# yweweler/single-speaker-tts

Hardware: AMD Instinct MI355X
Metric: mel-frames/sec (end-to-end text->waveform incl. 60-iter Griffin-Lim, 64-utt LJ-Speech-shaped batch per GPU) (higher is better)
Workload: dtype f32

## Files before the change

single-speaker-tts_amd/csrc/api_handle.hip:

```cpp
#include "api_internal.h"

namespace tts_api {
thread_local std::string g_create_error;
const char* const kStageNames[ST_COUNT] = {"encoder", "decoder", "postnet", "denorm", "gl_iter", "gl_final", "debug_gemm", "eval_loss", "features"};
}

namespace tts_api {


int fail(tts_handle_t h, int code, const std::string& msg) {
    if (h) h->err = msg;
    else g_create_error = msg;
    return code;
}


const char* kAtt = "decoder2/decoder/output_projection_wrapper/multi_rnn_cell/cell_0/attention_wrapper";

const char* kMrc = "decoder2/decoder/output_projection_wrapper/multi_rnn_cell";


std::string bn_name(int i) {
    return i == 0 ? std::string("batch_normalization") : "batch_normalization_" + std::to_string(i);
}
// ... 571 lines not shown
        if (h->hio.ids_dev[i]) hipFree(h->hio.ids_dev[i]);
        if (h->hio.wav_pinned[i]) hipHostFree(h->hio.wav_pinned[i]);
        if (h->hio.wav_dev[i]) hipFree(h->hio.wav_dev[i]);
        if (i == 0) {
            for (auto& kv : h->glg.tw) hipFree(kv.second);
            if (h->glg.window) hipFree(h->glg.window);
            if (h->glg.rwss) hipFree(h->glg.rwss);
        }
        if (h->hio.lin_pinned[i]) hipHostFree(h->hio.lin_pinned[i]);
        if (h->hio.lin_dev[i]) hipFree(h->hio.lin_dev[i]);
        if (h->hio.ali_pinned[i]) hipHostFree(h->hio.ali_pinned[i]);
        if (h->hio.ali_dev[i]) hipFree(h->hio.ali_dev[i]);
        if (h->hio.ev_h2d[i]) hipEventDestroy(h->hio.ev_h2d[i]);
        if (h->hio.ev_enc[i]) hipEventDestroy(h->hio.ev_enc[i]);
        if (h->hio.ev_ready[i]) hipEventDestroy(h->hio.ev_ready[i]);
        if (h->hio.ev_d2h[i]) hipEventDestroy(h->hio.ev_d2h[i]);
    }
    if (h->hio.status_pinned) hipHostFree(h->hio.status_pinned);
    if (h->hio.out) hipStreamDestroy(h->hio.out);
    if (h->ev_aux) hipEventDestroy(h->ev_aux);
    if (h->ev_front_done) hipEventDestroy(h->ev_front_done);
    for (int i = 0; i < 2; ++i) {
        if (h->ev_enc_ready[i]) hipEventDestroy(h->ev_enc_ready[i]);
        if (h->ev_dec_done[i]) hipEventDestroy(h->ev_dec_done[i]);
        if (h->ev_gap[i]) hipEventDestroy(h->ev_gap[i]);
    }
    if (h->encs) hipStreamDestroy(h->encs);
    if (h->ev_serial_done) hipEventDestroy(h->ev_serial_done);
    if (h->ev_graph_done) hipEventDestroy(h->ev_graph_done);
    for (int i = 0; i < 2; ++i) {
        if (h->ev_post_done[i]) hipEventDestroy(h->ev_post_done[i]);
        if (h->ev_gl_done[i]) hipEventDestroy(h->ev_gl_done[i]);
    }
    if (h->own_stream) hipStreamDestroy(h->stream);
    delete h;
    return TTS_OK;
}


const char* tts_last_error(tts_handle_t h) { return h ? h->err.c_str() : g_create_error.c_str(); }


int tts_set_stream(tts_handle_t h, void* s) {
    DeviceScope dev_scope(h);
    if (!h) return TTS_ERR_INVALID;
    {
        int rc = sync_all(h);
        if (rc) return rc;
    }
    h->post_pending[0] = h->post_pending[1] = false;
    h->gl_pending[0] = h->gl_pending[1] = false;
    h->gl_wide_used[0] = h->gl_wide_used[1] = false;
    {
        int rc = graph_drop(h);
        if (rc) return rc;
    }
    if (h->own_stream) hipStreamDestroy(h->stream);
    if (s) {
        h->stream = reinterpret_cast<hipStream_t>(s);
        h->own_stream = false;
    } else {
        HIPCHK(h, hipStreamCreate(&h->stream));
        h->own_stream = true;
    }
    return TTS_OK;
}


int tts_set_option(tts_handle_t h, const char* key, int value) {
    DeviceScope dev_scope(h);
    if (!h || !key) return TTS_ERR_INVALID;
    if (!std::strcmp(key, "use_graph")) {
        int have = 0;
        if (value && !(value == 2 && h->debug_hooks) && !graph_runtime_ok(&have))
            return fail(h, TTS_ERR_UNSUPPORTED,
                        "use_graph: this process runs the library on HIP runtime " + std::to_string(have) + ", older than the " +
                        std::to_string(HIP_VERSION) + " it was built with (a libamdhip64 loaded before the library, e.g. the one "
                        "PyTorch bundles); hipGraph replays of the decoder are wrong there (csrc/api_internal.h, `use_graph`) -- the "
                        "launches are enqueued directly instead");
        h->use_graph = value;
    }
    else if (!std::strcmp(key, "profile")) h->profile = value;
    else if (!std::strcmp(key, "fused_tail")) h->fused_tail = value;
    else if (!std::strcmp(key, "persistent_decoder")) {
        if (value != h->persistent_decoder) {
            int rc = sync_all(h);
            if (rc) return rc;
        }
        h->persistent_decoder = value;
    }
    else if (!std::strcmp(key, "gl_pair")) h->gl_pair = value;
    else if (!std::strcmp(key, "gl_wide_from")) h->gl_wide = value < -2 ? -2 : value;
    else if (!std::strcmp(key, "pd_ws")) {
        if (value != h->pd_ws) {
            int rc = sync_all(h);
            if (rc) return rc;
        }
        h->pd_ws = value;
    }
    else if (!std::strcmp(key, "enc_stream")) {
        int rc = sync_all(h);
        if (rc) return rc;
        h->enc_stream = value;
    }
    else if (!std::strcmp(key, "debug_hooks")) h->debug_hooks = value;
    else if (!std::strcmp(key, "pd_debug_delay") || !std::strcmp(key, "gl_runs") || !std::strcmp(key, "gl_run_len") ||
             !std::strcmp(key, "timeline") || !std::strcmp(key, "gl_workers") || !std::strcmp(key, "pd_rows")) {
        if (!h->debug_hooks && value != 0)
            return fail(h, TTS_ERR_INVALID, std::string(key) + ": a test hook; set the option \"debug_hooks\" to 1 on this handle first");
        if (!std::strcmp(key, "pd_debug_delay")) h->pd_debug_delay = value;
        else if (!std::strcmp(key, "gl_runs")) h->gl_runs = value;
        else if (!std::strcmp(key, "gl_run_len")) h->gl_run_len = value;
        else if (!std::strcmp(key, "gl_workers")) h->gl_workers = value;
        else if (!std::strcmp(key, "pd_rows")) h->pd_rows = value;
        else h->timeline = value;
    }
    else if (!std::strcmp(key, "reserve_cus")) {
        if (value != h->reserve_cus) {
            int rc = sync_all(h);
            if (rc) return rc;
        }
        h->reserve_cus = value;
    } else if (!std::strcmp(key, "hold_lds_kb")) {
        if (value < 1 || value > 160) return fail(h, TTS_ERR_INVALID, "hold_lds_kb must be 1..160");
        h->hold_lds_kb = value;
    } else if (!std::strcmp(key, "pipeline")) {
        int rc = sync_all(h);
        if (rc) return rc;
        h->post_pending[0] = h->post_pending[1] = false;
        h->gl_pending[0] = h->gl_pending[1] = false;
        h->gl_wide_used[0] = h->gl_wide_used[1] = false;
        h->pipeline = value;
    }
    else return fail(h, TTS_ERR_INVALID, std::string("unknown option ") + key);
    return TTS_OK;
}


int tts_synchronize(tts_handle_t h) {
    DeviceScope dev_scope(h);
    if (!h) return TTS_ERR_INVALID;
    return sync_all(h);
}


int tts_manifest_size(tts_handle_t h) { return h ? (int)h->manifest.size() : TTS_ERR_INVALID; }


int tts_manifest_entry(tts_handle_t h, int i, const char** name, int64_t shape[4], int* ndim) {
    if (!h || i < 0 || i >= (int)h->manifest.size()) return TTS_ERR_INVALID;
    const auto& e = h->manifest[i];
    if (name) *name = e.name.c_str();
    if (ndim) *ndim = (int)e.shape.size();
    if (shape)
        for (size_t d = 0; d < 4; ++d) shape[d] = d < e.shape.size() ? e.shape[d] : 1;
    return TTS_OK;
}


int tts_set_weight(tts_handle_t h, const char* name, const float* data, const int64_t* shape, int ndim) {
    if (!h || !name || !data || !shape) return TTS_ERR_INVALID;
    for (const auto& e : h->manifest) {
        if (e.name != name) continue;
        if ((int)e.shape.size() != ndim) return fail(h, TTS_ERR_INVALID, std::string("rank mismatch for ") + name);
        for (int d = 0; d < ndim; ++d)
            if (e.shape[d] != shape[d]) return fail(h, TTS_ERR_INVALID, std::string("shape mismatch for ") + name);
// ... 280 lines not shown
```

single-speaker-tts_amd/csrc/api_internal.h:

```cpp
#pragma once
#include <cmath>
#include <cstdio>
#include <cstring>
#include <memory>
#include <mutex>
#include <string>
#include <utility>
#include <vector>
#include "decoder.h"
#include "griffin_lim.h"
#include "tts_common.h"
#include <algorithm>
#include <map>

namespace tts_api {
using namespace tts;


extern thread_local std::string g_create_error;

struct ManifestEntry {
    std::string name;
    std::vector<int64_t> shape;
    size_t numel() const {
        size_t n = 1;
        for (auto d : shape) n *= (size_t)d;
        return n;
    }
};

struct CbhgWeights {
    int n_banks = 0, n_filters = 0, c_in = 0, proj_filters[2] = {0, 0};
    std::vector<const float*> bank_wt, bank_b, bank_scale, bank_shift;
    const float* proj_wt[2];
    const float* proj_b[2];
    const float* proj_scale[2];
    const float* proj_shift[2];
    const float* lifter_wt;
    const float* lifter_b;
    std::vector<const float*> hw_wt, hw_b;
    const float* gru_in_wt;
    const float* gru_in_b;
    const float* gru_rec;
};

enum Stage { ST_ENCODER = 0, ST_DECODER, ST_POSTNET, ST_DENORM, ST_GL_ITER, ST_GL_FINAL, ST_DEBUG_GEMM, ST_EVAL_LOSS, ST_FEATURES, ST_COUNT };
extern const char* const kStageNames[ST_COUNT];

struct ProfSpan {
    hipEvent_t a, b;
    int stage;
    int64_t launches;
};


}
using namespace tts_api;

struct tts_handle_s {
    tts_config_t cfg;
    int device = 0;
    hipStream_t stream = nullptr;
    bool own_stream = false;
    std::string err;
    int use_graph = 0;
    int fused_tail = 1;
    bool tail_configured = false;
    int profile = 0;
    int pipeline = 1;
    int reserve_cus = 32;
    int hold_lds_kb = 64;
    hipStream_t aux = nullptr;
    int* hold_flags = nullptr;
    hipEvent_t ev_aux = nullptr;
    unsigned call_count = 0;
    hipStream_t front = nullptr;
    hipStream_t encs = nullptr;
    int enc_stream = 1;
    hipEvent_t ev_enc_ready[2] = {nullptr, nullptr};
    hipEvent_t ev_dec_done[2] = {nullptr, nullptr};
    hipEvent_t ev_gap[2] = {nullptr, nullptr};
    bool enc_ready_pending[2] = {false, false}, dec_done_pending[2] = {false, false}, gap_pending[2] = {false, false};
    hipEvent_t ev_front_done = nullptr;
    hipEvent_t ev_post_done[2] = {nullptr, nullptr};
    bool post_pending[2] = {false, false};
    bool gl_wide_used[2] = {false, false};
    hipEvent_t ev_gl_done[2] = {nullptr, nullptr};
    bool gl_pending[2] = {false, false};
    bool front_pending = false;
    hipEvent_t ev_serial_done = nullptr;
    bool serial_pending = false;
    unsigned syn_calls = 0;
    int syn_shape[3] = {0, 0, 0};
    int last_enc_ahead = -1;
    bool in_synthesize = false;
    int persistent_decoder = 1;
    int pd_ws = 1;
    bool ws_configured = false;
    int gl_pair = 3;
    int gl_wide = -1;
    int n_cus_dev = 0;
    bool pd_configured = false;
    int debug_hooks = 0;
    int pd_debug_delay = 0;
    int gl_runs = 0;
    int gl_run_len = 0;
    int timeline = 0;
    int gl_workers = 0;
    unsigned* gl_ring = nullptr;
    unsigned gl_ring_seq = 0;
    unsigned* gl_ring_last = nullptr;
    hipStream_t gl_ring_stream = nullptr;
    float* pre_keys = nullptr;
    bool pd_used = false;
    unsigned* pd_sync = nullptr;
    int pd_clusters = 0;
    int* cur_hold_flag = nullptr;
    int cur_cu_budget = 0;
    bool dec_chip_idle = false;
    int pd_rows = 0;
    int pd_rows_used = 0;

    struct {
        hipStream_t out = nullptr;
        int32_t* ids_pinned[3] = {nullptr, nullptr, nullptr};
        int32_t* ids_dev[3] = {nullptr, nullptr, nullptr};
        size_t ids_bytes = 0;
        float* wav_dev[3] = {nullptr, nullptr, nullptr};
        float* wav_pinned[3] = {nullptr, nullptr, nullptr};
        size_t wav_bytes = 0;
        hipEvent_t ev_h2d[3] = {nullptr, nullptr, nullptr};
        hipEvent_t ev_enc[3] = {nullptr, nullptr, nullptr};
        hipEvent_t ev_ready[3] = {nullptr, nullptr, nullptr};
        hipEvent_t ev_d2h[3] = {nullptr, nullptr, nullptr};
        bool d2h_pending[3] = {false, false, false}, enc_pending[3] = {false, false, false};
        size_t n_floats[3] = {0, 0, 0};
        float* lin_dev[3] = {nullptr, nullptr, nullptr};
        float* lin_pinned[3] = {nullptr, nullptr, nullptr};
        size_t lin_bytes = 0;
        float* ali_dev[3] = {nullptr, nullptr, nullptr};
        float* ali_pinned[3] = {nullptr, nullptr, nullptr};
        size_t ali_bytes = 0;
        size_t n_lin[3] = {0, 0, 0}, n_ali[3] = {0, 0, 0};
        bool failed[3] = {false, false, false};
        int* status_pinned = nullptr;
        int tickets = 0;
    } hio;
    bool defer_projection = false, has_pending_proj = false;
    int defer_parity = 0;
// ... 189 lines not shown
```

single-speaker-tts_amd/csrc/api_stages.hip:

```cpp
#include "api_internal.h"

namespace tts_api {


int run_cbhg(tts_handle_t h, const CbhgWeights& w, const char* tag, const float* x, int B, int T, float* out,
             int64_t* launches) {
    const tts_config_t& c = h->cfg;
    const int M = B * T;
    const int NB = w.n_banks, NF = w.n_filters;
    const int U = c.n_highway_units, H = c.n_gru_units;
    const std::string t(tag);
    WS(h, (t + ".bank").c_str(), float, (size_t)M * NB * NF, bank);
    WS(h, (t + ".p1").c_str(), float, (size_t)M * w.proj_filters[0], p1);
    WS(h, (t + ".p2").c_str(), float, (size_t)M * w.proj_filters[1], p2);
    WS(h, (t + ".hw0").c_str(), float, (size_t)M * U, hw0);
    WS(h, (t + ".hw1").c_str(), float, (size_t)M * U, hw1);
    WS(h, (t + ".xproj").c_str(), float, (size_t)M * 6 * H, xproj);

    for (int k0 = 0; k0 < NB; k0 += TTS_GEMM_MAX_GROUPS) {
        GemmBatch b;
        std::memset(&b, 0, sizeof(b));
        const int ng = std::min(TTS_GEMM_MAX_GROUPS, NB - k0);
        for (int i = 0; i < ng; ++i) {
            const int k = k0 + ng - 1 - i;
            b.g[i] = conv_group(x, w.c_in, k + 1, T, w.bank_wt[k], w.bank_b[k], w.bank_scale[k], w.bank_shift[k], bank,
                                NB * NF, k * NF, M, NF, ACT_RELU, 0);
        }
        HIPCHK(h, launch_gemm(h->stream, b, ng));
        ++*launches;
    }
    {
        GemmGroup g = conv_group(bank, NB * NF, 3, T, w.proj_wt[0], w.proj_b[0], w.proj_scale[0], w.proj_shift[0], p1,
                                 w.proj_filters[0], 0, M, w.proj_filters[0], ACT_RELU, 1);
        const int slices = gemm_splitk_slices(g.K);
        if (slices > 1) {
            WS(h, (t + ".splitk").c_str(), float, (size_t)slices * M * g.N, part);
            HIPCHK(h, launch_gemm_splitk(h->stream, g, slices, part));
            ++*launches;
        } else {
            int rc = run_single(h, g);
            if (rc) return rc;
        }
        ++*launches;
    }
    {
        GemmGroup g = conv_group(p1, w.proj_filters[0], 3, T, w.proj_wt[1], w.proj_b[1], w.proj_scale[1],
                                 w.proj_shift[1], p2, w.proj_filters[1], 0, M, w.proj_filters[1], ACT_NONE, 0);
        g.R = x;
        g.ldr = w.c_in;
        int rc = run_single(h, g);
        if (rc) return rc;
        ++*launches;
    }
    if (h->fused_tail && cbhg_tail_supports(w.proj_filters[1], U, H, (int)w.hw_wt.size(), M)) {
        if (!h->tail_configured) {
            HIPCHK(h, cbhg_tail_configure());
            h->tail_configured = true;
        }
        CbhgTailParams tp;
        std::memset(&tp, 0, sizeof(tp));
        tp.X = p2; tp.ldx = w.proj_filters[1]; tp.c_in = w.proj_filters[1];
        tp.lifter_wt = w.lifter_wt; tp.lifter_b = w.lifter_b;
        tp.n_hw = (int)w.hw_wt.size();
        for (int l = 0; l < tp.n_hw; ++l) { tp.hw_wt[l] = w.hw_wt[l]; tp.hw_b[l] = w.hw_b[l]; }
        tp.gru_wt = w.gru_in_wt; tp.gru_b = w.gru_in_b;
        tp.hw_out = hw0; tp.xproj = xproj; tp.M = M;
        HIPCHK(h, launch_cbhg_tail(h->stream, tp));
        ++*launches;
    } else {
        {
            int rc = run_single(h, dense_group(p2, w.proj_filters[1], w.lifter_wt, w.lifter_b, hw0, U, M, U,
                                               w.proj_filters[1], ACT_RELU));
            if (rc) return rc;
            ++*launches;
        }
        float* cur = hw0;
        float* nxt = hw1;
        for (size_t l = 0; l < w.hw_wt.size(); ++l) {
            GemmGroup g = dense_group(cur, U, w.hw_wt[l], w.hw_b[l], nxt, U, M, 2 * U, U, ACT_NONE);
            g.epi = EPI_HIGHWAY;
            int rc = run_single(h, g);
            if (rc) return rc;
            ++*launches;
            std::swap(cur, nxt);
        }
        {
            int rc = run_single(h, dense_group(cur, U, w.gru_in_wt, w.gru_in_b, xproj, 6 * H, M, 6 * H, U, ACT_NONE));
            if (rc) return rc;
            ++*launches;
        }
    }
    HIPCHK(h, launch_bigru(h->stream, xproj, 6 * H, w.gru_rec, out, B, T, H, c.force_cudnn));
    ++*launches;
    return TTS_OK;
}


int check_ready(tts_handle_t h) {
    if (!h) return TTS_ERR_INVALID;
    if (!h->finalized) return fail(h, TTS_ERR_NOT_LOADED, "weights not loaded: call tts_finalize_weights first");
    return TTS_OK;
}


int gl_tables(tts_handle_t h) {
    auto& g = h->gl;
    if (g.configured) return TTS_OK;
    HIPCHK(h, gl_configure());
    std::vector<float2> t1(1024), t2(1024);
    for (int k = 0; k < 1024; ++k) {
        const double a1 = -2.0 * M_PI * k / 1024.0, a2 = -2.0 * M_PI * k / 2048.0;
        t1[k] = make_float2((float)std::cos(a1), (float)std::sin(a1));
        t2[k] = make_float2((float)std::cos(a2), (float)std::sin(a2));
    }
    HIPCHK(h, hipMalloc(&g.tw1024, 1024 * sizeof(float2)));
    HIPCHK(h, hipMalloc(&g.tw2048, 1024 * sizeof(float2)));
    HIPCHK(h, hipMemcpy(g.tw1024, t1.data(), 1024 * sizeof(float2), hipMemcpyHostToDevice));
    HIPCHK(h, hipMemcpy(g.tw2048, t2.data(), 1024 * sizeof(float2), hipMemcpyHostToDevice));
    {
        std::vector<float2> tb(1024 + 15 * 64);
        for (int k = 0; k < 1024; ++k) tb[k] = t2[k];
        for (int i = 0; i < 15 * 64; ++i) tb[1024 + i] = t1[(i & 63) * ((i >> 6) + 1)];
        HIPCHK(h, hipMalloc(&g.tables, tb.size() * sizeof(float2)));
        HIPCHK(h, hipMemcpy(g.tables, tb.data(), tb.size() * sizeof(float2), hipMemcpyHostToDevice));
    }
    {
        hipDeviceProp_t prop;
        HIPCHK(h, hipGetDeviceProperties(&prop, h->device));
        g.n_cus = prop.multiProcessorCount > 0 ? prop.multiProcessorCount : 256;
    }
    g.configured = true;
    return TTS_OK;
}


int device_cus(tts_handle_t h) { return h->gl.n_cus; }


int gl_fp(int n_fft);

int glg_prepare(tts_handle_t h, int T, int win, int hop, int n_fft);

int glg_twiddles(tts_handle_t h, int n_fft, const float2** out);


int stft_prepare(tts_handle_t h, int n, int win, int hop, int n_fft) {
    if (n_fft != TTS_GL_NFFT) return fail(h, TTS_ERR_UNSUPPORTED, "stft: n_fft != 2048 takes the general kernels (stft_run)");
    if (win < 2 || win > n_fft || hop < 1) return fail(h, TTS_ERR_INVALID, "stft: need 2 <= win_length <= n_fft, hop >= 1");
    if (n <= n_fft / 2) return fail(h, TTS_ERR_INVALID, "stft: signal shorter than n_fft/2 (reflect padding undefined)");
// ... 951 lines not shown
```

single-speaker-tts_amd/csrc/cbhg_tail.hip:

```cpp
#include "tts_common.h"

namespace tts {

#define CT_BM 128
#define CT_U 128
#define CT_XLD (CT_U + 4)
#define CT_BK 32
#define CT_BLD (CT_BK + 4)
#define CT_BN 256
#define CT_THREADS 512

#define CT_AIMG (3 * CT_BM * 64)
#define CT_BIMG (3 * CT_BN * 64)
size_t cbhg_tail_lds_bytes() { return (size_t)CT_BM * CT_XLD * sizeof(float) + CT_AIMG + CT_BIMG; }
typedef __bf16 ct_bf16x8_t __attribute__((ext_vector_type(8)));
__device__ __forceinline__ void ct_split3(float x, unsigned& h, unsigned& m, unsigned& l) {
    h = __float_as_uint(x);
    const float r1 = x - __uint_as_float(h & 0xFFFF0000u);
    m = __float_as_uint(r1);
    const float r2 = r1 - __uint_as_float(m & 0xFFFF0000u);
    l = __float_as_uint(r2);
}
__device__ __forceinline__ unsigned ct_pack_hi(unsigned a, unsigned b) { return __builtin_amdgcn_perm(b, a, 0x07060302u); }
__device__ __forceinline__ void ct_store_split4(unsigned char* img, int rows, int row, int kq, float4 v) {
    unsigned h[4], m[4], l[4];
    ct_split3(v.x, h[0], m[0], l[0]);
    ct_split3(v.y, h[1], m[1], l[1]);
    ct_split3(v.z, h[2], m[2], l[2]);
    ct_split3(v.w, h[3], m[3], l[3]);
    const int off = (row * 4 + ((kq >> 1) ^ ((row >> 2) & 3))) * 16 + (kq & 1) * 8;
    *reinterpret_cast<uint2*>(img + off) = make_uint2(ct_pack_hi(h[0], h[1]), ct_pack_hi(h[2], h[3]));
    *reinterpret_cast<uint2*>(img + rows * 64 + off) = make_uint2(ct_pack_hi(m[0], m[1]), ct_pack_hi(m[2], m[3]));
    *reinterpret_cast<uint2*>(img + 2 * rows * 64 + off) = make_uint2(ct_pack_hi(l[0], l[1]), ct_pack_hi(l[2], l[3]));
}

bool cbhg_tail_supports(int c_in, int units, int gru_units, int n_hw, long long M) {
    return units == CT_U && gru_units == 128 && c_in >= 4 && c_in <= CT_U && c_in % 4 == 0 && n_hw >= 0 && n_hw <= CBHG_TAIL_MAX_HW &&
           M >= 1 && (M + CT_BM) * 3 * CT_BN * (long long)sizeof(float) < 0xFFFFFFF0ll;
}

__global__ __launch_bounds__(CT_THREADS) void cbhg_tail_kernel(CbhgTailParams p) {
    extern __shared__ __attribute__((aligned(16))) float lds[];
    float* Xs = lds;
    unsigned char* Ai = reinterpret_cast<unsigned char*>(lds + CT_BM * CT_XLD);
    unsigned char* Bi = Ai + CT_AIMG;
    const int tid = threadIdx.x, lane = tid & 63, wave = tid >> 6;
    const int wm = wave & 1, wn = wave >> 1;
    const int li = lane & 31, lh = lane >> 5;
    const int m0 = blockIdx.x * CT_BM;
    const int M = p.M;

    {
        const __amdgpu_buffer_rsrc_t rs = __builtin_amdgcn_make_buffer_rsrc(const_cast<float*>(p.X), 0, (int)0xFFFFFFF0u, 0x00020000);
#pragma unroll
        for (int i = 0; i < (CT_BM * (CT_U / 4)) / CT_THREADS; ++i) {
            const int idx = tid + CT_THREADS * i;
            const int row = idx >> 5, c4 = idx & 31;
            const bool ok = m0 + row < M && 4 * c4 < p.c_in;
            const unsigned off = ok ? (unsigned)((size_t)(m0 + row) * p.ldx + 4 * c4) * 4u : 0xFFFFFFFFu;
            const float4 v = __builtin_bit_cast(float4, __builtin_amdgcn_raw_buffer_load_b128(rs, (int)off, 0, 0));
            *reinterpret_cast<float4*>(&Xs[row * CT_XLD + 4 * c4]) = v;
        }
    }

    const int n_jobs = 1 + p.n_hw + 3;
    const int kq = tid & 7;
    float4 rb[4];
    auto job_w = [&](int j) -> const float* {
        return j == 0 ? p.lifter_wt : (j <= p.n_hw ? p.hw_wt[j - 1] : p.gru_wt + (size_t)(j - 1 - p.n_hw) * CT_BN * CT_U);
    };
    auto job_k = [&](int j) { return j == 0 ? p.c_in : CT_U; };
    auto job_n = [&](int j) { return j == 0 ? CT_U : CT_BN; };
    auto load_chunk = [&](int j, int kc) {
        const __amdgpu_buffer_rsrc_t rs = __builtin_amdgcn_make_buffer_rsrc(const_cast<float*>(job_w(j)), 0, (int)0xFFFFFFF0u, 0x00020000);
        const int K = job_k(j), N = job_n(j);
        const int kk = kc * CT_BK + 4 * kq;
#pragma unroll
        for (int i = 0; i < 4; ++i) {
            const int row = (tid >> 3) + 64 * i;
            const bool ok = row < N && kk < K;
            rb[i] = __builtin_bit_cast(float4, __builtin_amdgcn_raw_buffer_load_b128(rs, ok ? (int)((unsigned)(row * K + kk) * 4u) : -1, 0, 0));
        }
    };
    auto stage_chunk = [&](int kc) {
#pragma unroll
        for (int i = 0; i < 4; ++i) ct_store_split4(Bi, CT_BN, (tid >> 3) + 64 * i, kq, rb[i]);
#pragma unroll
        for (int i = 0; i < 2; ++i) {
            const int row = (tid >> 3) + 64 * i;
            ct_store_split4(Ai, CT_BM, row, kq, *reinterpret_cast<const float4*>(&Xs[row * CT_XLD + kc * CT_BK + 4 * kq]));
        }
    };

    const __amdgpu_buffer_rsrc_t xp_rs = __builtin_amdgcn_make_buffer_rsrc(
        p.xproj, 0, (int)(unsigned)((size_t)M * 3 * CT_BN * sizeof(float) < 0xFFFFFFF0ull ? (size_t)M * 3 * CT_BN * sizeof(float) : 0xFFFFFFF0ull), 0x00020000);
    const __amdgpu_buffer_rsrc_t hw_rs = __builtin_amdgcn_make_buffer_rsrc(
        p.hw_out, 0, p.hw_out ? (int)(unsigned)((size_t)M * CT_U * sizeof(float)) : 0, 0x00020000);
    const int row_l = wm * 64 + 4 * lh;

    f32x16 acc[2][2];
    load_chunk(0, 0);
    for (int j = 0; j < n_jobs; ++j) {
        const int nch = (job_k(j) + CT_BK - 1) / CT_BK;
        const bool live = 64 * wn < job_n(j);
#pragma unroll
        for (int a = 0; a < 2; ++a)
#pragma unroll
            for (int b = 0; b < 2; ++b)
#pragma unroll
                for (int r = 0; r < 16; ++r) acc[a][b][r] = 0.f;
        for (int kc = 0; kc < nch; ++kc) {
            __syncthreads();
            stage_chunk(kc);
            __syncthreads();
            if (kc + 1 < nch) load_chunk(j, kc + 1);
            else if (j + 1 < n_jobs) load_chunk(j + 1, 0);
            if (live) {
#pragma unroll
                for (int q = 0; q < 2; ++q) {
                    const int ch = 2 * q + lh;
                    uint4 fa[2][3];
#pragma unroll
                    for (int tm = 0; tm < 2; ++tm) {
                        const int row = wm * 64 + tm * 32 + li;
                        const int off = (row * 4 + (ch ^ ((row >> 2) & 3))) * 16;
#pragma unroll
                        for (int sp = 0; sp < 3; ++sp) fa[tm][sp] = *reinterpret_cast<const uint4*>(Ai + sp * CT_BM * 64 + off);
                    }
#pragma unroll
                    for (int tn = 0; tn < 2; ++tn) {
                        const int row = wn * 64 + tn * 32 + li;
                        const int off = (row * 4 + (ch ^ ((row >> 2) & 3))) * 16;
                        uint4 fb[3];
#pragma unroll
                        for (int sp = 0; sp < 3; ++sp) fb[sp] = *reinterpret_cast<const uint4*>(Bi + sp * CT_BN * 64 + off);
#pragma unroll
                        for (int tm = 0; tm < 2; ++tm) {
#define CT_MMA(SA, SB)                                                                                                   \
                            acc[tm][tn] = __builtin_amdgcn_mfma_f32_32x32x16_bf16(__builtin_bit_cast(ct_bf16x8_t, fa[tm][SA]), \
                                                                                  __builtin_bit_cast(ct_bf16x8_t, fb[SB]), acc[tm][tn], 0, 0, 0);
                            CT_MMA(0, 2) CT_MMA(2, 0) CT_MMA(1, 1) CT_MMA(0, 1) CT_MMA(1, 0) CT_MMA(0, 0)
#undef CT_MMA
                        }
                    }
                }
            }
        }

        if (j == 0) {
            if (live) {
#pragma unroll
                for (int tn = 0; tn < 2; ++tn) {
                    const float b = p.lifter_b[wn * 64 + tn * 32 + li];
#pragma unroll
                    for (int tm = 0; tm < 2; ++tm)
#pragma unroll
                        for (int r = 0; r < 16; ++r) acc[tm][tn][r] = fmaxf(acc[tm][tn][r] + b, 0.f);
                }
            }
            __syncthreads();
            if (live) {
#pragma unroll
                for (int tn = 0; tn < 2; ++tn)
#pragma unroll
                    for (int tm = 0; tm < 2; ++tm)
#pragma unroll
                        for (int r = 0; r < 16; ++r) {
                            const int ro = tm * 32 + (r & 3) + 8 * (r >> 2);
                            Xs[(row_l + ro) * CT_XLD + wn * 64 + tn * 32 + li] = acc[tm][tn][r];
                        }
            }
        } else if (j <= p.n_hw) {
            const int unit = wn * 32 + li;
            const float bh = p.hw_b[j - 1][wn * 64 + li], bt = p.hw_b[j - 1][wn * 64 + 32 + li];
#pragma unroll
            for (int tm = 0; tm < 2; ++tm)
#pragma unroll
                for (int r = 0; r < 16; ++r) {
                    const int ro = tm * 32 + (r & 3) + 8 * (r >> 2);
                    const float hh = fmaxf(acc[tm][0][r] + bh, 0.f);
                    const float tt = sigmoidf_(acc[tm][1][r] + bt);
                    const float x = Xs[(row_l + ro) * CT_XLD + unit];
                    acc[tm][0][r] = hh * tt + x * (1.0f - tt);
                }
            __syncthreads();
#pragma unroll
            for (int tm = 0; tm < 2; ++tm)
#pragma unroll
                for (int r = 0; r < 16; ++r) {
                    const int ro = tm * 32 + (r & 3) + 8 * (r >> 2);
                    Xs[(row_l + ro) * CT_XLD + unit] = acc[tm][0][r];
                }
            if (j == p.n_hw) {
                const unsigned vb = (unsigned)((m0 + row_l) * CT_U + unit) * 4u;
#pragma unroll
                for (int tm = 0; tm < 2; ++tm)
#pragma unroll
                    for (int r = 0; r < 16; ++r) {
                        const int ro = tm * 32 + (r & 3) + 8 * (r >> 2);
                        const float y = acc[tm][0][r];
                        __builtin_amdgcn_raw_buffer_store_b32(__builtin_bit_cast(unsigned, y), hw_rs, (int)(vb + (unsigned)(ro * CT_U * 4)), 0, 0);
                    }
            }
        } else {
            const int pass = j - 1 - p.n_hw;
#pragma unroll
            for (int tn = 0; tn < 2; ++tn) {
                const int n = pass * CT_BN + wn * 64 + tn * 32 + li;
                const float b = p.gru_b[n];
                const unsigned vb = (unsigned)((m0 + row_l) * (3 * CT_BN) + n) * 4u;
#pragma unroll
                for (int tm = 0; tm < 2; ++tm)
#pragma unroll
                    for (int r = 0; r < 16; ++r) {
                        const int ro = tm * 32 + (r & 3) + 8 * (r >> 2);
                        const float y = acc[tm][tn][r] + b;
                        __builtin_amdgcn_raw_buffer_store_b32(__builtin_bit_cast(unsigned, y), xp_rs,
                                                              (int)(vb + (unsigned)(ro * 3 * CT_BN * 4)), 0, 0);
                    }
            }
        }
    }
    if (p.n_hw == 0 && p.hw_out) {
        __syncthreads();
        for (int idx = tid; idx < CT_BM * (CT_U / 4); idx += CT_THREADS) {
            const int row = idx >> 5, c4 = idx & 31;
            if (m0 + row < M)
                *reinterpret_cast<float4*>(&p.hw_out[(size_t)(m0 + row) * CT_U + 4 * c4]) = *reinterpret_cast<const float4*>(&Xs[row * CT_XLD + 4 * c4]);
        }
    }
}

hipError_t cbhg_tail_configure() {
    return hipFuncSetAttribute(reinterpret_cast<const void*>(&cbhg_tail_kernel), hipFuncAttributeMaxDynamicSharedMemorySize,
                               (int)cbhg_tail_lds_bytes());
}

hipError_t launch_cbhg_tail(hipStream_t s, const CbhgTailParams& p) {
    if (p.M < 1) return hipSuccess;
    hipLaunchKernelGGL(cbhg_tail_kernel, dim3((p.M + CT_BM - 1) / CT_BM), dim3(CT_THREADS), cbhg_tail_lds_bytes(), s, p);
    return hipGetLastError();
}

}
```

single-speaker-tts_amd/csrc/gru.hip:

```cpp
#include "tts_common.h"

namespace tts {

#define GRU_THREADS 512
#define GRU_QPAD 36

template <int CTRL>
__device__ __forceinline__ float gru_dpp(float v) {
    return __builtin_bit_cast(float, __builtin_amdgcn_update_dpp(0, __builtin_bit_cast(int, v), CTRL, 0xF, 0xF, true));
}
__device__ __forceinline__ float gru_sum4(float v) {
    v += gru_dpp<0xB1>(v);
    v += gru_dpp<0x4E>(v);
    return v;
}
__device__ __forceinline__ void gru_lds_barrier() { asm volatile("s_waitcnt lgkmcnt(0)\n\ts_barrier" ::: "memory"); }
typedef float gru_f2 __attribute__((ext_vector_type(2)));
__device__ __forceinline__ gru_f2 gru_pk_fma(gru_f2 a, gru_f2 b, gru_f2 c) {
    gru_f2 d;
    asm("v_pk_fma_f32 %0, %1, %2, %3" : "=v"(d) : "v"(a), "v"(b), "v"(c));
    return d;
}
__device__ __forceinline__ float gru_dot32(const float* q, const gru_f2 (&w)[16]) {
    gru_f2 a = {0.f, 0.f}, b = {0.f, 0.f};
#pragma unroll
    for (int i = 0; i < 32; i += 4) {
        const float4 hv = *reinterpret_cast<const float4*>(q + i);
        a = gru_pk_fma((gru_f2){hv.x, hv.y}, w[i / 2], a);
        b = gru_pk_fma((gru_f2){hv.z, hv.w}, w[i / 2 + 1], b);
    }
    return (a.x + a.y) + (b.x + b.y);
}

template <int H, bool CUDNN>
__global__ __launch_bounds__(GRU_THREADS) void bigru_kernel(const float* __restrict__ xproj, int xld,
                                                            const float* __restrict__ wrec,
                                                            float* __restrict__ out, int B, int T) {
    static_assert(H == 128, "thread mapping assumes 128 units");
    const int b = blockIdx.x;
    const int d = blockIdx.y;
    const int tid = threadIdx.x;
    const int j = tid >> 2, kq = tid & 3;

    __shared__ __attribute__((aligned(16))) float hs[2][4 * GRU_QPAD];
    __shared__ __attribute__((aligned(16))) float rhs[4 * GRU_QPAD];

    const size_t wstride = (size_t)H * 2 * H + (size_t)H * H + (CUDNN ? H : 0);
    const float* wg_g = wrec + d * wstride;
    const float* wc_g = wg_g + (size_t)H * 2 * H;
    const float* bch_g = wc_g + (size_t)H * H;

    gru_f2 wr[16], wu[16], wc[16];
#pragma unroll
    for (int i = 0; i < 16; ++i) {
        const size_t k0 = 32 * kq + 2 * i;
        wr[i] = (gru_f2){wg_g[k0 * (2 * H) + j], wg_g[(k0 + 1) * (2 * H) + j]};
        wu[i] = (gru_f2){wg_g[k0 * (2 * H) + H + j], wg_g[(k0 + 1) * (2 * H) + H + j]};
        wc[i] = (gru_f2){wc_g[k0 * H + j], wc_g[(k0 + 1) * H + j]};
    }
    float bch = 0.f;
    if (CUDNN) bch = bch_g[j];

    if (tid < 4 * GRU_QPAD) { hs[0][tid] = 0.f; hs[1][tid] = 0.f; rhs[tid] = 0.f; }
    __syncthreads();

    const float* xb = xproj + (size_t)b * T * xld + (size_t)d * 3 * H + j;
    float* ob = out + (size_t)b * T * 2 * H + (size_t)d * H + j;
    const int slot = (j >> 5) * GRU_QPAD + (j & 31);

    int t = d ? T - 1 : 0;
    const int dt = d ? -1 : 1;
    auto xrow = [&](int s) {
        const int sc = s < T ? s : T - 1;
        return xb + (size_t)(d ? T - 1 - sc : sc) * xld;
    };
    float xa[3] = {xrow(0)[0], xrow(0)[H], xrow(0)[2 * H]};
    float xb1[3] = {xrow(1)[0], xrow(1)[H], xrow(1)[2 * H]};
    float xc2[3] = {xrow(2)[0], xrow(2)[H], xrow(2)[2 * H]};
    float hreg = 0.f;

    int s = 0;
#define GRU_STEP(X)                                                                            \
    {                                                                                          \
        const float* hq = hs[s & 1] + kq * GRU_QPAD;                                           \
        const float r = sigmoidf_(X[0] + gru_sum4(gru_dot32(hq, wr)));                         \
        const float u = sigmoidf_(X[1] + gru_sum4(gru_dot32(hq, wu)));                         \
        float c;                                                                               \
        if (CUDNN) {  \
            c = tanhf_(X[2] + r * (gru_sum4(gru_dot32(hq, wc)) + bch));                        \
        } else {                                                                               \
            if (kq == 0) rhs[slot] = r * hreg;                                                 \
            gru_lds_barrier();                                                                 \
            c = tanhf_(X[2] + gru_sum4(gru_dot32(rhs + kq * GRU_QPAD, wc)));                   \
        }                                                                                      \
        hreg = u * hreg + (1.0f - u) * c;                                                      \
        if (kq == 0) {                                                                         \
            ob[(size_t)t * 2 * H] = hreg;                                                      \
            hs[(s + 1) & 1][slot] = hreg;                                                      \
        }                                                                                      \
        const float* xn = xrow(s + 3);                                                         \
        X[0] = xn[0]; X[1] = xn[H]; X[2] = xn[2 * H];                                          \
        ++s; t += dt;                                                                          \
        gru_lds_barrier();                                                                     \
    }
    while (s + 3 <= T) {
        GRU_STEP(xa)
        GRU_STEP(xb1)
        GRU_STEP(xc2)
    }
    if (s < T) GRU_STEP(xa)
    if (s < T) GRU_STEP(xb1)
#undef GRU_STEP
}

size_t bigru_wrec_floats(int H, int cudnn) {
    return 2 * ((size_t)H * 2 * H + (size_t)H * H + (cudnn ? H : 0));
}

hipError_t launch_bigru(hipStream_t s, const float* xproj, int xld, const float* wrec, float* out,
                        int B, int T, int H, int cudnn) {
    if (H != 128) return hipErrorInvalidValue;
    dim3 grid(B, 2);
    if (cudnn)
        hipLaunchKernelGGL((bigru_kernel<128, true>), grid, dim3(GRU_THREADS), 0, s, xproj, xld, wrec, out, B, T);
    else
        hipLaunchKernelGGL((bigru_kernel<128, false>), grid, dim3(GRU_THREADS), 0, s, xproj, xld, wrec, out, B, T);
    return hipGetLastError();
}

}
```

single-speaker-tts_amd/csrc/tts_common.h:

```cpp
#pragma once
#include <hip/hip_runtime.h>
#include <stdint.h>
#include <stddef.h>
#include <map>
#include <string>
#include <vector>

#include "../../include/sstts_hip.h"

namespace tts {

typedef float f32x4 __attribute__((ext_vector_type(4)));
typedef float f32x16 __attribute__((ext_vector_type(16)));

enum Act { ACT_NONE = 0, ACT_RELU = 1, ACT_SIGMOID = 2, ACT_TANH = 3 };
enum Epi { EPI_STD = 0, EPI_HIGHWAY = 1 };

__device__ __forceinline__ float sigmoidf_(float x) { return __builtin_amdgcn_rcpf(1.0f + __expf(-x)); }
__device__ __forceinline__ double wave_sum_f64(double v) {
#pragma unroll
    for (int o = 32; o > 0; o >>= 1) v += __shfl_xor(v, o);
    return v;
}
__device__ __forceinline__ void split_f64(double v, float* hi, float* lo) {
    *hi = (float)v;
    *lo = (float)(v - (double)*hi);
}
__device__ __forceinline__ float predicted_centre(double z, int Ts) {
    const float zf = (float)z;
    const double e = (double)expf(-zf) * (1.0 - (z - (double)zf));
    return (float)((double)Ts / (1.0 + e));
}

__device__ __forceinline__ float tanhf_(float x) {
    float e = __expf(2.0f * x);
    return fmaf(-2.0f, __builtin_amdgcn_rcpf(e + 1.0f), 1.0f);
}
__device__ __forceinline__ float clip_keep_nan(float x, float lo, float hi) {
    const float c = fminf(fmaxf(x, lo), hi);
    return x != x ? x : c;
}
__device__ __forceinline__ float denorm_db(float x, float ref_db, float range_db) {
    const float c = clip_keep_nan(x, 0.f, 1.f);
    return (c - 1.0f) * range_db + ref_db;
}
__device__ __forceinline__ float db_pow(float db, float power) {
    return exp2f(db * (power * (0.05f * 3.3219280948873623f)));
}
__device__ __forceinline__ float denorm_pow(float x, float ref_db, float range_db, float power) {
    return db_pow(denorm_db(x, ref_db, range_db), power);
}
__device__ __forceinline__ float apply_act(float v, int act) {
    if (act == ACT_RELU) return fmaxf(v, 0.0f);
    if (act == ACT_SIGMOID) return sigmoidf_(v);
    if (act == ACT_TANH) return tanhf_(v);
    return v;
}

struct GemmGroup {
    const float* A;
    const int32_t* gather;
    int gather_rows;
    const float* Wt;
    const float* bias;
    const float* scale;
    const float* shift;
    const float* R;
    float* C;
    int M, N, K;
    int lda, T, Cin, padl, pool;
    int ldc, coff, ldr;
    int act, epi;
    float* C2;
    int ldc2, N2;
    float d_ref, d_range, d_pow;
    int* d_flag;
    int kt0, kt1;
};
#define TTS_GEMM_MAX_GROUPS 16
struct GemmBatch {
    GemmGroup g[TTS_GEMM_MAX_GROUPS];
};
hipError_t launch_gemm(hipStream_t s, const GemmBatch& b, int n_groups);
hipError_t launch_gemm_splitk(hipStream_t s, const GemmGroup& g, int slices, float* partial);
int gemm_splitk_slices(int K);

hipError_t launch_bigru(hipStream_t s, const float* xproj, int xld, const float* wrec, float* out,
                        int B, int T, int H, int cudnn);
size_t bigru_wrec_floats(int H, int cudnn);

#define CBHG_TAIL_MAX_HW 8
struct CbhgTailParams {
    const float* X; int ldx; int c_in;
    const float* lifter_wt; const float* lifter_b;
    const float* hw_wt[CBHG_TAIL_MAX_HW]; const float* hw_b[CBHG_TAIL_MAX_HW]; int n_hw;
    const float* gru_wt; const float* gru_b;
    float* hw_out;
    float* xproj;
    int M;
};
bool cbhg_tail_supports(int c_in, int units, int gru_units, int n_hw, long long M);
hipError_t cbhg_tail_configure();
hipError_t launch_cbhg_tail(hipStream_t s, const CbhgTailParams& p);

hipError_t cu_hold_configure();
hipError_t launch_cu_hold(hipStream_t s, int n_cus, const int* flag, double timeout_ms, int lds_kb = 64);

size_t eval_loss_partial_count(int B, int T, int n_mels, int F);
hipError_t launch_eval_loss(hipStream_t s, const float* mel_t, const float* mel_o, const float* lin_t, const float* lin_o, int B,
                            int T, int n_mels, int F, int max_blocks, double* partial, double* sums, float* losses);

struct DevBuf {
    void* p = nullptr;
    size_t bytes = 0;
};

}
```

Measured before the change: 4.418 million.

## Fold CBHG second projection conv into fused tail kernel

Adds a templated FOLD path to the fused CBHG tail kernel. It runs the second projection conv (3-tap over p1, plus bias, batch-norm scale/shift and the residual from x) as an extra leading GEMM job inside the tail kernel, so p2 is never written to global memory except for debugging. This removes one kernel launch and a round trip of p2 through global memory, at the cost of more kernel complexity and a per-row tap mask for sequence boundaries. The GRU x-prefetch loop is also refactored into a generic compile-time prefetch depth, kept at 3.

```diff
diff --git a/single-speaker-tts_amd/csrc/api_handle.hip b/single-speaker-tts_amd/csrc/api_handle.hip
--- a/single-speaker-tts_amd/csrc/api_handle.hip
+++ b/single-speaker-tts_amd/csrc/api_handle.hip
@@ -677,6 +677,7 @@
     }
     else if (!std::strcmp(key, "profile")) h->profile = value;
     else if (!std::strcmp(key, "fused_tail")) h->fused_tail = value;
+    else if (!std::strcmp(key, "tail_proj2")) h->tail_proj2 = value;
     else if (!std::strcmp(key, "persistent_decoder")) {
         if (value != h->persistent_decoder) {
             int rc = sync_all(h);
diff --git a/single-speaker-tts_amd/csrc/api_internal.h b/single-speaker-tts_amd/csrc/api_internal.h
--- a/single-speaker-tts_amd/csrc/api_internal.h
+++ b/single-speaker-tts_amd/csrc/api_internal.h
@@ -65,6 +65,7 @@
     std::string err;
     int use_graph = 0;
     int fused_tail = 1;
+    int tail_proj2 = 1;
     bool tail_configured = false;
     int profile = 0;
     int pipeline = 1;
diff --git a/single-speaker-tts_amd/csrc/api_stages.hip b/single-speaker-tts_amd/csrc/api_stages.hip
--- a/single-speaker-tts_amd/csrc/api_stages.hip
+++ b/single-speaker-tts_amd/csrc/api_stages.hip
@@ -43,7 +43,10 @@
         }
         ++*launches;
     }
-    {
+    const bool tail = h->fused_tail && cbhg_tail_supports(w.proj_filters[1], U, H, (int)w.hw_wt.size(), M);
+    const bool fold = tail && h->tail_proj2 && w.c_in == w.proj_filters[1] &&
+                      cbhg_tail_supports(w.proj_filters[1], U, H, (int)w.hw_wt.size(), M, w.proj_filters[0], T);
+    if (!fold) {
         GemmGroup g = conv_group(p1, w.proj_filters[0], 3, T, w.proj_wt[1], w.proj_b[1], w.proj_scale[1],
                                  w.proj_shift[1], p2, w.proj_filters[1], 0, M, w.proj_filters[1], ACT_NONE, 0);
         g.R = x;
@@ -52,7 +55,7 @@
         if (rc) return rc;
         ++*launches;
     }
-    if (h->fused_tail && cbhg_tail_supports(w.proj_filters[1], U, H, (int)w.hw_wt.size(), M)) {
+    if (tail) {
         if (!h->tail_configured) {
             HIPCHK(h, cbhg_tail_configure());
             h->tail_configured = true;
@@ -65,6 +68,12 @@
         for (int l = 0; l < tp.n_hw; ++l) { tp.hw_wt[l] = w.hw_wt[l]; tp.hw_b[l] = w.hw_b[l]; }
         tp.gru_wt = w.gru_in_wt; tp.gru_b = w.gru_in_b;
         tp.hw_out = hw0; tp.xproj = xproj; tp.M = M;
+        if (fold) {
+            tp.P1 = p1; tp.c1 = w.proj_filters[0]; tp.T = T;
+            tp.p2_wt = w.proj_wt[1]; tp.p2_b = w.proj_b[1]; tp.p2_scale = w.proj_scale[1]; tp.p2_shift = w.proj_shift[1];
+            tp.X = x; tp.ldx = w.c_in;
+            tp.p2_out = (!h->in_synthesize || h->debug_hooks) ? p2 : nullptr;
+        }
         HIPCHK(h, launch_cbhg_tail(h->stream, tp));
         ++*launches;
     } else {
diff --git a/single-speaker-tts_amd/csrc/cbhg_tail.hip b/single-speaker-tts_amd/csrc/cbhg_tail.hip
--- a/single-speaker-tts_amd/csrc/cbhg_tail.hip
+++ b/single-speaker-tts_amd/csrc/cbhg_tail.hip
@@ -34,11 +34,15 @@
     *reinterpret_cast<uint2*>(img + 2 * rows * 64 + off) = make_uint2(ct_pack_hi(l[0], l[1]), ct_pack_hi(l[2], l[3]));
 }
 
-bool cbhg_tail_supports(int c_in, int units, int gru_units, int n_hw, long long M) {
-    return units == CT_U && gru_units == 128 && c_in >= 4 && c_in <= CT_U && c_in % 4 == 0 && n_hw >= 0 && n_hw <= CBHG_TAIL_MAX_HW &&
-           M >= 1 && (M + CT_BM) * 3 * CT_BN * (long long)sizeof(float) < 0xFFFFFFF0ll;
-}
-
+bool cbhg_tail_supports(int c_in, int units, int gru_units, int n_hw, long long M, int c1, int T) {
+    const bool tail = units == CT_U && gru_units == 128 && c_in >= 4 && c_in <= CT_U && c_in % 4 == 0 && n_hw >= 0 &&
+                      n_hw <= CBHG_TAIL_MAX_HW && M >= 1 && (M + CT_BM) * 3 * CT_BN * (long long)sizeof(float) < 0xFFFFFFF0ll;
+    if (c1 <= 0) return tail;
+    return tail && c1 % CT_BK == 0 && T >= 1 && M % T == 0 && (M + 1) * (long long)c1 * (long long)sizeof(float) < 0xFFFFFFF0ll &&
+           3ll * c1 * c_in * (long long)sizeof(float) < 0xFFFFFFF0ll;
+}
+
+template <bool FOLD>
 __global__ __launch_bounds__(CT_THREADS) void cbhg_tail_kernel(CbhgTailParams p) {
     extern __shared__ __attribute__((aligned(16))) float lds[];
     float* Xs = lds;
@@ -63,18 +67,44 @@
         }
     }
 
-    const int n_jobs = 1 + p.n_hw + 3;
+    constexpr int J0 = FOLD ? -1 : 0;
+    const int j_end = 1 + p.n_hw + 3;
     const int kq = tid & 7;
     float4 rb[4];
+    float4 ra[2];
+    unsigned a_taps[2];
+    if (FOLD) {
+#pragma unroll
+        for (int i = 0; i < 2; ++i) {
+            const int m = m0 + (tid >> 3) + 64 * i;
+            const int t = m % p.T;
+            a_taps[i] = m < M ? ((t > 0 ? 1u : 0u) | 2u | (t < p.T - 1 ? 4u : 0u)) : 0u;
+        }
+    }
+    const __amdgpu_buffer_rsrc_t p1_rs = __builtin_amdgcn_make_buffer_rsrc(const_cast<float*>(p.P1), 0, (int)0xFFFFFFF0u, 0x00020000);
     auto job_w = [&](int j) -> const float* {
+        if (FOLD && j < 0) return p.p2_wt;
         return j == 0 ? p.lifter_wt : (j <= p.n_hw ? p.hw_wt[j - 1] : p.gru_wt + (size_t)(j - 1 - p.n_hw) * CT_BN * CT_U);
     };
-    auto job_k = [&](int j) { return j == 0 ? p.c_in : CT_U; };
-    auto job_n = [&](int j) { return j == 0 ? CT_U : CT_BN; };
+    auto job_k = [&](int j) { return FOLD && j < 0 ? 3 * p.c1 : (j == 0 ? p.c_in : CT_U); };
+    auto job_n = [&](int j) { return FOLD && j < 0 ? p.c_in : (j == 0 ? CT_U : CT_BN); };
     auto load_chunk = [&](int j, int kc) {
         const __amdgpu_buffer_rsrc_t rs = __builtin_amdgcn_make_buffer_rsrc(const_cast<float*>(job_w(j)), 0, (int)0xFFFFFFF0u, 0x00020000);
         const int K = job_k(j), N = job_n(j);
-        const int kk = kc * CT_BK + 4 * kq;
+        int kk = kc * CT_BK + 4 * kq;
+        if (FOLD) {
+            const bool proj = j < 0;
+            const int cc = kc / 3, tap = kc - 3 * cc;
+            const int ch = cc * CT_BK + 4 * kq;
+            if (proj) kk = tap * p.c1 + ch;
+#pragma unroll
+            for (int i = 0; i < 2; ++i) {
+                const int m = m0 + (tid >> 3) + 64 * i;
+                const bool ok = proj && ((a_taps[i] >> tap) & 1u);
+                ra[i] = __builtin_bit_cast(float4, __builtin_amdgcn_raw_buffer_load_b128(
+                                                       p1_rs, ok ? (int)((unsigned)((m - 1 + tap) * p.c1 + ch) * 4u) : -1, 0, 0));
+            }
+        }
 #pragma unroll
         for (int i = 0; i < 4; ++i) {
             const int row = (tid >> 3) + 64 * i;
@@ -82,7 +112,14 @@
             rb[i] = __builtin_bit_cast(float4, __builtin_amdgcn_raw_buffer_load_b128(rs, ok ? (int)((unsigned)(row * K + kk) * 4u) : -1, 0, 0));
         }
     };
-    auto stage_chunk = [&](int kc) {
+    auto stage_chunk = [&](int j, int kc) {
+        if (FOLD && j < 0) {
+#pragma unroll
+            for (int i = 0; i < 2; ++i) ct_store_split4(Bi, CT_BN, (tid >> 3) + 64 * i, kq, rb[i]);
+#pragma unroll
+            for (int i = 0; i < 2; ++i) ct_store_split4(Ai, CT_BM, (tid >> 3) + 64 * i, kq, ra[i]);
+            return;
+        }
 #pragma unroll
         for (int i = 0; i < 4; ++i) ct_store_split4(Bi, CT_BN, (tid >> 3) + 64 * i, kq, rb[i]);
 #pragma unroll
@@ -99,10 +136,11 @@
     const int row_l = wm * 64 + 4 * lh;
 
     f32x16 acc[2][2];
-    load_chunk(0, 0);
-    for (int j = 0; j < n_jobs; ++j) {
+    load_chunk(J0, 0);
+    for (int j = J0; j < j_end; ++j) {
         const int nch = (job_k(j) + CT_BK - 1) / CT_BK;
         const bool live = 64 * wn < job_n(j);
+        const bool live1 = !FOLD || 64 * wn + 32 < job_n(j);
 #pragma unroll
         for (int a = 0; a < 2; ++a)
 #pragma unroll
@@ -111,10 +149,10 @@
                 for (int r = 0; r < 16; ++r) acc[a][b][r] = 0.f;
         for (int kc = 0; kc < nch; ++kc) {
             __syncthreads();
-            stage_chunk(kc);
+            stage_chunk(j, kc);
             __syncthreads();
             if (kc + 1 < nch) load_chunk(j, kc + 1);
-            else if (j + 1 < n_jobs) load_chunk(j + 1, 0);
+            else if (j + 1 < j_end) load_chunk(j + 1, 0);
             if (live) {
 #pragma unroll
                 for (int q = 0; q < 2; ++q) {
@@ -129,6 +167,7 @@
                     }
 #pragma unroll
                     for (int tn = 0; tn < 2; ++tn) {
+                        if (FOLD && tn == 1 && !live1) continue;
                         const int row = wn * 64 + tn * 32 + li;
                         const int off = (row * 4 + (ch ^ ((row >> 2) & 3))) * 16;
                         uint4 fb[3];
@@ -147,7 +186,40 @@
             }
         }
 
-        if (j == 0) {
+        if (FOLD && j < 0) {
+            if (live) {
+                const int N = p.c_in;
+#pragma unroll
+                for (int tn = 0; tn < 2; ++tn) {
+                    const int n = wn * 64 + tn * 32 + li;
+                    if (n < N) {
+                        const float bv = p.p2_b[n];
+                        const float sc = p.p2_scale ? p.p2_scale[n] : 1.f;
+                        const float sh = p.p2_scale ? p.p2_shift[n] : 0.f;
+#pragma unroll
+                        for (int tm = 0; tm < 2; ++tm)
+#pragma unroll
+                            for (int r = 0; r < 16; ++r) {
+                                const int ro = tm * 32 + (r & 3) + 8 * (r >> 2);
+                                float v = acc[tm][tn][r] + bv;
+                                v = v * sc + sh;
+                                v += Xs[(row_l + ro) * CT_XLD + n];
+                                Xs[(row_l + ro) * CT_XLD + n] = v;
+                            }
+                    }
+                }
+            }
+            if (p.p2_out) {
+                __syncthreads();
+                const int n4 = p.c_in >> 2;
+                for (int idx = tid; idx < CT_BM * n4; idx += CT_THREADS) {
+                    const int row = idx / n4, c4 = idx - row * n4;
+                    if (m0 + row < M)
+                        *reinterpret_cast<float4*>(&p.p2_out[(size_t)(m0 + row) * p.c_in + 4 * c4]) =
+                            *reinterpret_cast<const float4*>(&Xs[row * CT_XLD + 4 * c4]);
+                }
+            }
+        } else if (j == 0) {
             if (live) {
 #pragma unroll
                 for (int tn = 0; tn < 2; ++tn) {
@@ -232,13 +304,18 @@
 }
 
 hipError_t cbhg_tail_configure() {
-    return hipFuncSetAttribute(reinterpret_cast<const void*>(&cbhg_tail_kernel), hipFuncAttributeMaxDynamicSharedMemorySize,
+    hipError_t e = hipFuncSetAttribute(reinterpret_cast<const void*>(&cbhg_tail_kernel<false>),
+                                       hipFuncAttributeMaxDynamicSharedMemorySize, (int)cbhg_tail_lds_bytes());
+    if (e != hipSuccess) return e;
+    return hipFuncSetAttribute(reinterpret_cast<const void*>(&cbhg_tail_kernel<true>), hipFuncAttributeMaxDynamicSharedMemorySize,
                                (int)cbhg_tail_lds_bytes());
 }
 
 hipError_t launch_cbhg_tail(hipStream_t s, const CbhgTailParams& p) {
     if (p.M < 1) return hipSuccess;
-    hipLaunchKernelGGL(cbhg_tail_kernel, dim3((p.M + CT_BM - 1) / CT_BM), dim3(CT_THREADS), cbhg_tail_lds_bytes(), s, p);
+    const dim3 grid((p.M + CT_BM - 1) / CT_BM);
+    if (p.P1) hipLaunchKernelGGL(cbhg_tail_kernel<true>, grid, dim3(CT_THREADS), cbhg_tail_lds_bytes(), s, p);
+    else hipLaunchKernelGGL(cbhg_tail_kernel<false>, grid, dim3(CT_THREADS), cbhg_tail_lds_bytes(), s, p);
     return hipGetLastError();
 }
 
diff --git a/single-speaker-tts_amd/csrc/gru.hip b/single-speaker-tts_amd/csrc/gru.hip
--- a/single-speaker-tts_amd/csrc/gru.hip
+++ b/single-speaker-tts_amd/csrc/gru.hip
@@ -1,9 +1,13 @@
 #include "tts_common.h"
+#include <type_traits>
 
 namespace tts {
 
 #define GRU_THREADS 512
 #define GRU_QPAD 36
+#ifndef GRU_PREFETCH
+#define GRU_PREFETCH 3
+#endif
 
 template <int CTRL>
 __device__ __forceinline__ float gru_dpp(float v) {
@@ -30,6 +34,14 @@
         b = gru_pk_fma((gru_f2){hv.z, hv.w}, w[i / 2 + 1], b);
     }
     return (a.x + a.y) + (b.x + b.y);
+}
+
+template <int I, int N, class F>
+__device__ __forceinline__ void gru_static_for(F&& f) {
+    if constexpr (I < N) {
+        f(std::integral_constant<int, I>{});
+        gru_static_for<I + 1, N>(f);
+    }
 }
 
 template <int H, bool CUDNN>
@@ -70,13 +82,16 @@
 
     int t = d ? T - 1 : 0;
     const int dt = d ? -1 : 1;
+    constexpr int D = GRU_PREFETCH;
     auto xrow = [&](int s) {
         const int sc = s < T ? s : T - 1;
         return xb + (size_t)(d ? T - 1 - sc : sc) * xld;
     };
-    float xa[3] = {xrow(0)[0], xrow(0)[H], xrow(0)[2 * H]};
-    float xb1[3] = {xrow(1)[0], xrow(1)[H], xrow(1)[2 * H]};
-    float xc2[3] = {xrow(2)[0], xrow(2)[H], xrow(2)[2 * H]};
+    float x[D][3];
+    gru_static_for<0, D>([&](auto ic) {
+        constexpr int i = decltype(ic)::value;
+        x[i][0] = xrow(i)[0]; x[i][1] = xrow(i)[H]; x[i][2] = xrow(i)[2 * H];
+    });
     float hreg = 0.f;
 
     int s = 0;
@@ -98,18 +113,15 @@
             ob[(size_t)t * 2 * H] = hreg;                                                      \
             hs[(s + 1) & 1][slot] = hreg;                                                      \
         }                                                                                      \
-        const float* xn = xrow(s + 3);                                                         \
+        const float* xn = xrow(s + D);                                                         \
         X[0] = xn[0]; X[1] = xn[H]; X[2] = xn[2 * H];                                          \
         ++s; t += dt;                                                                          \
         gru_lds_barrier();                                                                     \
     }
-    while (s + 3 <= T) {
-        GRU_STEP(xa)
-        GRU_STEP(xb1)
-        GRU_STEP(xc2)
-    }
-    if (s < T) GRU_STEP(xa)
-    if (s < T) GRU_STEP(xb1)
+    while (s + D <= T) gru_static_for<0, D>([&](auto ic) { GRU_STEP(x[decltype(ic)::value]) });
+    gru_static_for<0, D - 1>([&](auto ic) {
+        if (s < T) GRU_STEP(x[decltype(ic)::value])
+    });
 #undef GRU_STEP
 }
 
diff --git a/single-speaker-tts_amd/csrc/tts_common.h b/single-speaker-tts_amd/csrc/tts_common.h
--- a/single-speaker-tts_amd/csrc/tts_common.h
+++ b/single-speaker-tts_amd/csrc/tts_common.h
@@ -98,8 +98,12 @@
     float* hw_out;
     float* xproj;
     int M;
+    const float* P1; int c1; int T;
+    const float* p2_wt;
+    const float* p2_b; const float* p2_scale; const float* p2_shift;
+    float* p2_out;
 };
-bool cbhg_tail_supports(int c_in, int units, int gru_units, int n_hw, long long M);
+bool cbhg_tail_supports(int c_in, int units, int gru_units, int n_hw, long long M, int c1 = 0, int T = 0);
 hipError_t cbhg_tail_configure();
 hipError_t launch_cbhg_tail(hipStream_t s, const CbhgTailParams& p);
 
```

Result: no change. 4.450 million (median of 6 runs) (+0.7%).
